# matyasosvath/hutoken

Hardware: AMD Instinct MI355X
Metric: GB/s input text encoded (GPT-2 vocab) at 1/2/4/8 GPUs; bit-exact ids (higher is better)
Workload: dtype u8

## Files before the change

hutoken_amd/_capi.py:

```python
import ctypes as C
import importlib.util
import os
import sys

from . import build as _build

OK = 0
E_FILE_NOT_FOUND, E_VALUE, E_MEMORY, E_ARG, E_DEVICE, E_UNSUPPORTED = 1, 2, 3, 4, 5, 6
E_CAPACITY, E_NUL_BYTE, E_WORD_TOO_LARGE, E_INVALID_UTF8 = 7, 8, 9, 10
DOC_OK, DOC_WORD_TOO_LARGE, DOC_INVALID_UTF8 = 0, 1, 2
DOC_ID_OUT_OF_RANGE, DOC_ID_UNDECODABLE, DOC_SPAN_MISMATCH = 3, 4, 5

_vp, _i64, _i32, _s32, _u32, _str = C.c_void_p, C.c_int64, C.c_int, C.c_int32, C.c_uint32, C.c_char_p
_pvp, _pi64, _ps32, _pf = C.POINTER(_vp), C.POINTER(_i64), C.POINTER(_s32), C.POINTER(C.c_float)
_DEV = [_vp, _vp, _vp, _i64, _i64, _vp, _i64, _vp, _vp, _vp, _vp]
_DEV_F = [_vp, _vp, _vp, _i64, _i64, _i32, _vp, _i64, _vp, _vp, _vp, _vp]
_HOST = [_vp, _vp, _vp, _i64, _vp, _i64, _vp, _vp]
_HOST_F = [_vp, _vp, _vp, _i64, _i32, _vp, _i64, _vp, _vp]
SIGNATURES = {
    "hutk_ctx_create": (_i32, [_pvp, _str, _str, _str, _i32, _i32]),
    "hutk_ctx_create_merges": (_i32, [_pvp, _str, _str, _str, _i32, _str, _i32]),
    "hutk_ctx_set_pattern": (_i32, [_vp, _str]),
    "hutk_ctx_set_pretokenizer": (_i32, [_vp, _i32, _vp, _i64]),
    "hutk_ctx_pretokenizer": (_i32, [_vp]),
    "hutk_ctx_add_device": (_i32, [_vp, _i32]),
    "hutk_ctx_device_count": (_i32, [_vp]),
    "hutk_uses_merges": (_i32, [_vp]),
    "hutk_ctx_destroy": (None, [_vp]),
    "hutk_last_error": (_str, []),
    "hutk_ids_capacity": (_i64, [_vp, _i64, _i64]),
    "hutk_encode_batch": (_i32, _HOST),
    "hutk_encode_batch_device": (_i32, _DEV),
    "hutk_encode": (_i32, [_vp, _vp, _i64, _vp, _i64, _pi64, _ps32]),
    "hutk_vocab_size": (_i64, [_vp]),
    "hutk_host_alloc": (_vp, [C.c_size_t]),
    "hutk_host_free": (None, [_vp]),
    "hutk_decode_batch": (_i32, _HOST),
    "hutk_decode_batch_device": (_i32, _DEV),
    "hutk_pair_table_entries": (_i64, [_vp]),
    "hutk_device_ordinal": (_i32, [_vp]),
    "hutk_table_stats": (_i32, [_vp, _vp]),
    "hutk_last_timing": (_i32, [_vp, _pf, _pf]),
    "hutk_set_timing": (None, [_vp, _i32]),
    "hutk_debug_pairs_second": (_i64, [_vp]),
    "hutk_debug_long_words": (_i64, [_vp]),
    "hutk_debug_profile": (_i32, [_vp, _i32]),
    "hutk_debug_profile_read": (_i32, [_vp, _i64, _vp]),
    "hutk_debug_profile_raw": (_i32, [_vp, _i64, _vp]),
    "hutk_debug_tile_bytes": (_i32, []),
    "hutk_debug_seam": (_i32, [_vp, _vp]),
    "hutk_debug_seam2_cut": (_i32, [_vp, _u32, _u32]),
    "hutk_debug_tile_kernel": (_i32, [_vp, _i64]),
    "hutk_debug_exc_counts": (_i32, [_vp, _vp]),
    "hutk_ctx_word_cache_stats": (_i32, [_vp, _vp]),
    "hutk_ctx_word_cache_clear": (_i32, [_vp]),
    "hutk_trainer_create": (_i32, [_pvp, _i32]),
    "hutk_trainer_add": (_i32, [_vp, _vp, _vp, _i64]),
    "hutk_trainer_run": (_i32, [_vp, _s32, _vp, _vp, _ps32]),
    "hutk_trainer_stats": (_i32, [_vp, _vp]),
    "hutk_trainer_destroy": (None, [_vp]),
    "hutk_trainer_debug_counters": (_i32, [_vp, _vp, _i32]),
    "hutk_trainer_create_mode": (_i32, [_pvp, _i32, _i32]),
    "hutk_trainer_alphabet": (_i32, [_vp, _vp, _i64, _vp, _i64, _pi64, _pi64]),
    "hutk_collate_padded_device": (_i32, [_vp, _vp, _i64, _i64, _i64, _s32, _s32, _s32, _i32, _i32, _vp, _vp, _vp, _vp, _vp]),
    "hutk_packer_create": (_i32, [_pvp, _i64, _s32, _s32, _s32, _i32, _i32]),
    "hutk_packer_rows": (_i64, [_vp, _i64, _i64]),
    "hutk_packer_add_device": (_i32, [_vp, _vp, _vp, _i64, _i64, _vp, _vp, _vp, _i64, _pi64, _vp, _vp]),
    "hutk_packer_flush_device": (_i32, [_vp, _vp, _vp, _vp, _pi64, _vp]),
    "hutk_packer_pending": (_i64, [_vp]),
    "hutk_packer_destroy": (None, [_vp]),
    "hutk_packer_create_channels": (_i32, [_pvp, _i64, _s32, _s32, _s32, _i32, _i32, _i32, _vp, _vp, _vp]),
    "hutk_packer_channel_count": (_i32, [_vp]),
    "hutk_packer_add_channels_device": (_i32, [_vp, _vp, _vp, _i64, _i64, _vp, _vp, _vp, _vp, _vp, _i64, _pi64, _vp, _vp]),
    "hutk_packer_flush_channels_device": (_i32, [_vp, _vp, _vp, _vp, _vp, _pi64, _vp]),
    "hutk_packed_cu_seqlens_device": (_i32, [_vp, _i64, _i64, _i64, _vp, _vp, _vp, _vp]),
    "hutk_packed_labels_device": (_i32, [_vp, _i32, _vp, _i64, _i64, _i32, _i64, _vp, _vp]),
    "hutk_debug_cu_tile": (_i32, []),
    "hutk_bestfit_rows_bound": (_i64, [_i64, _i64, _i64, _i32]),
# ... 272 lines not shown
        raise_for(load().hutk_ctx_set_pattern(self._h, None if pattern is None else pattern.encode("utf-8")))

    def set_pretokenizer(self, preset, blob=None):
        if preset is None:
            raise_for(load().hutk_ctx_set_pretokenizer(self._h, -1, None, 0))
            return
        buf = (C.c_uint8 * max(len(blob), 1)).from_buffer_copy(bytes(blob) or b"\0")
        raise_for(load().hutk_ctx_set_pretokenizer(self._h, int(preset), C.cast(buf, C.c_void_p), len(blob)))

    @property
    def pretokenizer(self):
        p = load().hutk_ctx_pretokenizer(self._h)
        return None if p < 0 else p

    @property
    def uses_merges(self):
        return bool(load().hutk_uses_merges(self._h))

    @property
    def handle(self):
        return self._h

    def ids_capacity(self, n_bytes, n_docs):
        return load().hutk_ids_capacity(self._h, n_bytes, n_docs)

    def table_stats(self):
        import numpy as np
        out = np.zeros(8, dtype=np.int64)
        raise_for(load().hutk_table_stats(self._h, out.ctypes.data))
        keys = ["n_keys", "n_vocab_sym", "n_sym", "n_pairs", "pair_slots", "rank_is_sym", "ident_ids", "n_word_entries"]
        d = dict(zip(keys, out.tolist()))
        if hasattr(load(), "hutk_debug_long_words"):
            d["n_long_word_entries"] = int(load().hutk_debug_long_words(self._h))
        return d

    def seam_map(self):
        import numpy as np
        out = np.zeros(256, dtype=np.uint32)
        on = load().hutk_debug_seam(self._h, out.ctypes.data)
        return out, bool(on)

    def seam2_cut(self, a3, b3):
        return bool(load().hutk_debug_seam2_cut(self._h, int.from_bytes(a3, "little"), int.from_bytes(b3, "little")))

    def tile_kernel(self, n_bytes):
        k = load().hutk_debug_tile_kernel(self._h, int(n_bytes))
        if k < 0:
            raise_for(E_ARG)
        return k

    def exc_counts(self):
        import numpy as np
        out = np.zeros(8, dtype=np.int64)
        raise_for(load().hutk_debug_exc_counts(self._h, out.ctypes.data))
        v = out.tolist()
        return {"exc": v[0], "lists": v[1:6], "tail": v[6], "has_multi": bool(v[7])}

    def word_cache_stats(self):
        import numpy as np
        out = np.zeros(4, dtype=np.int64)
        raise_for(load().hutk_ctx_word_cache_stats(self._h, out.ctypes.data))
        v = out.tolist()
        return {"entries": v[0], "capacity": v[1], "appended": v[2], "open": bool(v[3])}

    def word_cache_clear(self):
        raise_for(load().hutk_ctx_word_cache_clear(self._h))
# ... 816 lines not shown
```

hutoken_amd/csrc/hutk_api.cpp:

```cpp
#include <hip/hip_runtime.h>

#include <regex.h>
#if defined(__linux__)
#include <sys/syscall.h>
#include <unistd.h>
#endif

#include <algorithm>
#include <atomic>
#include <cctype>
#include <chrono>
#include <cstdio>
#include <cstdlib>
#include <cstring>
#include <mutex>
#include <new>
#include <string>
#include <thread>
#include <vector>

#include "hutk_classify.h"
#include "hutk_host.h"
constexpr int PTILES_DEFAULT = 2;

// ... 275 lines not shown
    const size_t n = T.cand_sym.size();
    if (!n) return HUTK_OK;
    std::vector<int64_t> offs(n + 1), oo(n + 1);
    for (size_t i = 0; i <= n; i++) offs[i] = T.cand_off[i];
    std::vector<int32_t> ids((size_t)hutk_ids_capacity(c, (int64_t)T.cand_bytes.size(), (int64_t)n));
    const int had_prefix = c->dt.has_prefix;
    c->dt.has_prefix = 0;
    int rc = hutk_encode_batch(c, T.cand_bytes.data(), offs.data(), (int64_t)n, ids.data(), (int64_t)ids.size(),
                               oo.data(), nullptr);
    c->dt.has_prefix = had_prefix;
    if (rc) return rc;
    const int64_t key_bytes = T.sym16 ? WORD_KEY_BYTES_16 : WORD_KEY_BYTES_32;
    std::vector<size_t> keep, keep_long;
    for (size_t i = 0; i < n; i++)
        if (oo[i + 1] - oo[i] == 1 && ids[oo[i]] == T.sym_id[T.cand_sym[i]] && offs[i + 1] - offs[i] >= 2 &&
            offs[i + 1] - offs[i] <= WORDL_KEY_BYTES)
            (offs[i + 1] - offs[i] <= key_bytes ? keep : keep_long).push_back(i);
    auto key_of = [&](size_t i, uint32_t* k) {
        for (int q = 0; q < 7; q++) k[q] = 0;
        const size_t len = (size_t)(offs[i + 1] - offs[i]);
        for (size_t j = 0; j < len; j++) k[j >> 2] |= (uint32_t)T.cand_bytes[offs[i] + j] << (8 * (j & 3));
    };
    std::vector<WordSlot> slots(1, WordSlot{{0, 0, 0, 0}});
    uint32_t cap = 0;
    if (!keep.empty()) {
        std::vector<uint4> kk(keep.size());
        for (size_t q = 0; q < keep.size(); q++) {
            uint32_t k[7];
            key_of(keep[q], k);
            kk[q] = make_uint4(k[0], k[1], k[2], k[3]);
        }
        cap = 1024;
        while (cap < keep.size() * 5 / 2 + 16) cap <<= 1;
        std::vector<uint32_t> where, homeless;
        auto hash_of = [&](uint32_t j) { const uint4 k = kk[j]; return word_hash(k.x, k.y, k.z, k.w); };
        cuckoo_place(keep.size(), cap, [&](uint32_t j) { return hash_of(j) & (cap - 1); },
                     [&](uint32_t j) { return word_slot2(hash_of(j), cap - 1); }, where, &homeless);
        slots.assign(cap + 1, WordSlot{{0, 0, 0, 0}});
        for (size_t j = 0; j < keep.size(); j++) {
            if (where[j] == 0xFFFFFFFFu) continue;
            const uint4 k = kk[j];
            slots[where[j]] = T.sym16 ? WordSlot{{k.x, k.y, k.z, k.w | (T.cand_sym[keep[j]] << 16)}}
                                      : WordSlot{{k.x, k.y, k.z, T.cand_sym[keep[j]]}};
            c->n_word_entries++;
        }
    }
    uint32_t lcap = 0, loff = 0;
    if (cap && !keep_long.empty() && !getenv("HUTK_NO_LONG_WORD_TABLE")) {
        lcap = 256;
        while (lcap < keep_long.size() * 8 + 16) lcap <<= 1;
        loff = (uint32_t)slots.size();
        loff += loff & 1u;
        slots.resize((size_t)loff + 2 * (size_t)lcap, WordSlot{{0, 0, 0, 0}});
        for (size_t j = 0; j < keep_long.size(); j++) {
            uint32_t k[7];
            key_of(keep_long[j], k);
            const size_t at = (size_t)loff + 2 * (size_t)(word_hash_long(k[0], k[1], k[2], k[3], k[4], k[5], k[6]) & (lcap - 1));
            if (slots[at].k[0] | slots[at].k[1] | slots[at].k[2] | slots[at].k[3]) continue;
            slots[at] = WordSlot{{k[0], k[1], k[2], k[3]}};
            slots[at + 1] = WordSlot{{k[4], k[5], k[6], T.cand_sym[keep_long[j]]}};
            c->n_word_entries++;
            c->n_wordl_entries++;
        }
    }
    if (!cap) return HUTK_OK;
    HUTK_HIP_TRY(c->d_word_tab.reserve(slots.size()));
    HUTK_HIP_TRY(hipMemcpy(c->d_word_tab.p, slots.data(), slots.size() * sizeof(WordSlot), hipMemcpyHostToDevice));
    c->dt.word_tab = c->d_word_tab.p;
    c->dt.word_mask = cap - 1;
    c->dt.wordl_off = loff;
// ... 113 lines not shown
        return rc;
    }
    p->pattern = c->pattern;
    if (c->presplit >= 0) {
        const int prc = hutk_pretokenizer_create(&p->pretok, device, c->presplit_blob.data(), (int64_t)c->presplit_blob.size());
        if (prc) {
            std::string keep = g_err;
            destroy(p);
            g_err = keep;
            return prc;
        }
        p->presplit = c->presplit;
    }
    c->peers.push_back(p);
    c->peer_ids.emplace_back();
    return HUTK_OK;
}

int hutk_ctx_device_count(const hutk_ctx* c) { return c && !c->host_only ? 1 + (int)c->peers.size() : 0; }

void hutk_ctx_destroy(hutk_ctx* ctx) { destroy(ctx); }

int64_t hutk_ids_capacity(const hutk_ctx* ctx, int64_t n_bytes, int64_t n_docs) {
    if (!ctx) return 0;
    return n_bytes * (int64_t)ctx->tab.max_units_per_item + (int64_t)pad_per_doc(ctx) * n_docs + 1;
}

int64_t hutk_vocab_size(const hutk_ctx* ctx) { return ctx ? ctx->tab.n_keys : 0; }
int hutk_uses_merges(const hutk_ctx* ctx) { return ctx && ctx->tab.id_path ? 1 : 0; }
int64_t hutk_pair_table_entries(const hutk_ctx* ctx) { return ctx ? ctx->tab.n_pairs : 0; }
int hutk_device_ordinal(const hutk_ctx* ctx) { return ctx ? ctx->device : -1; }
int64_t hutk_debug_pairs_second(const hutk_ctx* ctx) { return ctx ? ctx->tab.n_pairs_second : 0; }
int64_t hutk_debug_long_words(const hutk_ctx* ctx) { return ctx ? ctx->n_wordl_entries : 0; }
int hutk_debug_seam(const hutk_ctx* ctx, uint32_t* out256) {
    if (!ctx || !out256) return api_set_error(HUTK_E_ARG, "bad argument");
    memcpy(out256, ctx->tab.seam_hi, sizeof ctx->tab.seam_hi);
    return seams_wanted(ctx->tab) ? 1 : 0;
}
int hutk_debug_seam2_cut(const hutk_ctx* ctx, uint32_t a3, uint32_t b3) {
    if (!ctx) return 0;
    const Tables& T = ctx->tab;
    if (!T.seam_on || !T.seam2_on || (getenv("HUTK_NO_SEAM") && atoi(getenv("HUTK_NO_SEAM"))) ||
        (getenv("HUTK_NO_SEAM2") && atoi(getenv("HUTK_NO_SEAM2"))))
        return 0;
    if (!seam2_char3(a3) || !seam2_char3(b3)) return 0;
    if ((T.seam2_part[(a3 >> 16) & 0xFFu] >> (b3 & 31u)) & 1u) return 0;
    const uint32_t kinds[5][2] = {{3, 3}, {3, 2}, {3, 1}, {1, 3}, {1, 2}};
    for (auto& kk : kinds) {
        if (!(T.seam2_cats & seam2_cat_bit(kk[0], kk[1]))) continue;
        const uint32_t a = kk[0] == 3 ? a3 : (a3 >> 16) & 0xFFu;
        const uint32_t b = kk[1] == 3 ? b3 : kk[1] == 2 ? (b3 & 0xFFFFu) : (b3 & 0xFFu);
        const uint32_t h = seam2_hash(a, b, kk[0], kk[1]) >> T.seam2_shift;
        if ((T.seam2_bits[h >> 5] >> (h & 31)) & 1u) return 0;
    }
    return 1;
}
void hutk_set_timing(hutk_ctx* ctx, int enabled) {
    if (ctx) ctx->timing = enabled != 0;
}

int hutk_table_stats(const hutk_ctx* ctx, int64_t* out8) {
    if (!ctx || !out8) return HUTK_E_ARG;
    const Tables& T = ctx->tab;
    out8[0] = T.n_keys;
    out8[1] = T.n_vocab_sym;
    out8[2] = T.n_sym;
// ... 855 lines not shown
```

hutoken_amd/csrc/hutk_host.h:

```cpp
#pragma once
#include <hip/hip_runtime.h>

#include <mutex>
#include <string>
#include <utility>
#include <vector>

#include "hutk_device.h"

#define HUTK_HIP_TRY(expr)                                                                                  \
    do {                                                                                                    \
        hipError_t e__ = (expr);                                                                            \
        if (e__ != hipSuccess)                                                                              \
            return hutk::api_set_error(HUTK_E_DEVICE, std::string("HIP error: ") + hipGetErrorString(e__) + \
                                                          " at " #expr);                                    \
    } while (0)

namespace hutk {

template <class T>
struct DevBuf {
    T* p = nullptr;
    size_t cap = 0;
    hipError_t reserve(size_t n) {
// ... 47 lines not shown
        return HUTK_OK;
    }
    DecTables tables(bool skip) const {
        DecTables t{};
        t.ent = skip ? dx_ent_skip.p : dx_ent.p;
        t.sent = !strip ? nullptr : skip ? dx_sent_skip.p : dx_sent.p;
        t.blob = dx_blob.p;
        t.n = n;
        return t;
    }
    void release() {
        dx_ent.release(); dx_sent.release(); dx_ent_skip.release(); dx_sent_skip.release(); dx_slots.release();
        dx_blob.release();
    }
};

}

using hutk::DevBuf;

struct hutk_ctx {
    hutk::Tables tab;
    int device = -1;
    bool host_only = false;
    bool timing = true;

    DevBuf<uint64_t> d_pair, d_char;
    DevBuf<int32_t> d_sym_id, d_prefix_alone;
    DevBuf<uint32_t> d_item_sym, d_prefix_syms, d_prefix_alone_syms, d_seam, d_seam2, d_item_units;
    DevBuf<uint8_t> d_item_direct, d_split_dfa;
    DevBuf<uint32_t> d_bytepair16;
    DevBuf<hutk::WordSlot> d_word_tab;
    int64_t n_word_entries = 0, n_wordl_entries = 0;
    DevBuf<uint4> d_wc_tab, d_wc_list;
    DevBuf<uint32_t> d_wc_tags, d_wc_ctl;
    uint32_t wc_list_cap = 0;
    DevBuf<uint64_t> d_bytepair32;
    DevBuf<long long> w_prof;
    bool profile = false;
    std::string pattern;
    DevBuf<uint32_t> w_wbits, w_gbits, w_fbits, w_abits;
    int presplit = -1;
    struct hutk_pretokenizer* pretok = nullptr;
    std::vector<uint8_t> presplit_blob;
    hutk::DevTables dt{};

    DevBuf<uint32_t> w_run;
    DevBuf<int32_t> w_exc_tok;
    DevBuf<uint32_t> w_exc_sym, w_exc_mrg, w_tile_u32, w_doc_pos, w_counters;
    DevBuf<int64_t> w_tile_i64;
    DevBuf<hutk::ExcRec> w_exc;
    DevBuf<uint32_t> w_exc_quad, w_exc_mid, w_exc_wave;
    int last_tail = -1;

    DevBuf<uint2> d_dec_ent, d_dec_sent;
    DevBuf<uint8_t> d_dec_blob;
    hutk::DecTables dec{};
    DevBuf<uint32_t> dw_first;
    DevBuf<unsigned long long> dw_state;
    DevBuf<int64_t> dw_tfd;
    DevBuf<int32_t> dw_ids;
    DevBuf<int32_t> ds_ids, ds_status;
    DevBuf<int64_t> ds_offs, ds_oo;
    DevBuf<uint8_t> ds_bytes;
    DevBuf<int32_t> w_err;
    DevBuf<uint64_t> sp_bits;
// ... 270 lines not shown
```

hutoken_amd/csrc/hutk_internal.h:

```cpp
#pragma once
#include "hutk_seam2.h"
#include <cstdint>
#include <string>
#include <vector>

#include "hutoken_amd.h"

#if defined(__HIPCC__)
#include <hip/hip_runtime.h>
#define HUTK_HD __host__ __device__ __forceinline__
#else
#define HUTK_HD inline
#endif

namespace hutk {

constexpr uint32_t SYM_BITS = 20;
constexpr uint32_t SYM_UNK = (1u << SYM_BITS) - 1;
constexpr uint32_t SYM_NONE = 0xFFFFFFFFu;
constexpr uint64_t SLOT_EMPTY = ~0ull;
constexpr int WORDL_KEY_BYTES = 28;

constexpr uint32_t PAIR_ABSENT = 0xFFFFFu;
static inline uint64_t pair_slot(uint32_t l, uint32_t r, uint32_t m) {
// ... 36 lines not shown
                                std::vector<uint32_t>* failed = nullptr) {
    const uint32_t NONE = 0xFFFFFFFFu;
    std::vector<uint32_t> owner(cap, NONE);
    where.assign(n, NONE);
    bool all = true;
    uint64_t rng = 0x9E3779B97F4A7C15ull;
    for (size_t i = 0; i < n; i++) {
        uint32_t cur = (uint32_t)i;
        uint32_t slot = h1(cur) & (cap - 1);
        bool placed = false;
        for (int kick = 0; kick < 2000; kick++) {
            const uint32_t a = h1(cur) & (cap - 1), b = h2(cur) & (cap - 1);
            if (owner[a] == NONE) slot = a;
            else if (owner[b] == NONE) slot = b;
            else {
                rng = rng * 6364136223846793005ull + 1442695040888963407ull;
                slot = (slot == a) ? b : (slot == b) ? a : ((rng >> 33) & 1u ? a : b);
            }
            const uint32_t prev = owner[slot];
            owner[slot] = cur;
            where[cur] = slot;
            if (prev == NONE) { placed = true; break; }
            where[prev] = NONE;
            cur = prev;
        }
        if (!placed) {
            all = false;
            if (!failed) return false;
            failed->push_back(cur);
        }
    }
    return all;
}
HUTK_HD uint32_t char_hash(uint32_t packed) {
    uint32_t h = packed * 0x9E3779B1u;
    h ^= h >> 16;
    return h * 0x85EBCA6Bu;
}
HUTK_HD uint32_t char_slot1(uint32_t h, uint32_t shift) { return h >> shift; }
HUTK_HD uint32_t char_slot2(uint32_t h, uint32_t mask) { return ((h >> 7) ^ ((h & 0x7Fu) * 0x2F1Bu) ^ 0x5A5Au) & mask; }

constexpr int64_t MAX_WORD_BYTES = 262144;

struct Tables {
    int64_t n_keys = 0;
    uint32_t n_vocab_sym = 0;
    uint32_t n_sym = 0;
    bool rank_is_sym = false;
    bool ident_ids = false;
    std::vector<int32_t> sym_id;
    int32_t byte_tok[256] = {0};

    std::vector<uint64_t> pair_slots;
    uint32_t pair_shift = 0;
    int64_t n_pairs = 0;
    int64_t n_pairs_second = 0;

    uint32_t item_sym[256];
    uint8_t item_direct[256];
    uint32_t multi_bits[8] = {0, 0, 0, 0, 0, 0, 0, 0};
    uint32_t item_units_off[257] = {0};
    std::vector<uint32_t> item_units;
    uint32_t max_units_per_item = 1;
    bool has_multi = false;
    std::vector<uint64_t> char_slots;
    uint32_t char_mask = 0;
// ... 59 lines not shown
```

hutoken_amd/csrc/hutk_kernels.hip:

```cpp
#include <hip/hip_runtime.h>

#include <type_traits>

#include "hutk_kdev.h"
#include "hutk_lab.h"

namespace hutk {

__device__ __noinline__ void cut_note_cold(uint32_t* noreal_bits, uint32_t* counters, uint32_t tile, unsigned long long mine,
                                                  uint32_t last16, uint32_t* cutpos) {
    if ((threadIdx.x & 63) != 0) return;
    if (mine == 0) {
        atomicOr(&noreal_bits[tile >> 5], 1u << (tile & 31));
        atomicAdd(&counters[CTR_NOREAL_TILES], 1u);
    } else {
        *cutpos = 1u + (uint32_t)(16 * (63 - __builtin_clzll(mine)) + 31 - __builtin_clz(last16 & 0xFFFFu));
    }
}

struct Win8 { uint32_t d[8]; };
__device__ __noinline__ uint32_t classify16_exact_cold(Win8 w, uint32_t dbits, uint32_t* tmp) {
#pragma unroll
    for (int i = 0; i < 8; i++) tmp[i] = w.d[i];
    return classify16_exact(*reinterpret_cast<const uint32_t(*)[8]>(tmp), dbits);
// ... 46 lines not shown
template <typename SymT, bool BYTE_MODE>
struct TileLds {
    static constexpr int ARENA_WORDS = 4, ARENA_W = LANE_MAX_UNITS + 4;
    __attribute__((aligned(16))) uint8_t sb[WINDOW];
    uint32_t docm[WINDOW / 32 + 3];
    __attribute__((aligned(8))) uint16_t wmask16[64 + 8];
    __attribute__((aligned(8))) uint32_t mergem[NPOS / 32 + 2];
    __attribute__((aligned(8))) uint32_t excm[NPOS / 32 + 2];
    __attribute__((aligned(8))) uint32_t livem[NPOS / 32 + 2];
    uint16_t stage[64];
    __attribute__((aligned(16))) SymT S[NPOS];
    SymT arenaS[BYTE_MODE ? 1 : ARENA_WORDS * ARENA_W];
    SymT arenaM[BYTE_MODE ? 1 : ARENA_WORDS * ARENA_W];
    uint32_t arena_live[ARENA_WORDS];
    uint16_t arena_ws[ARENA_WORDS], arena_n[ARENA_WORDS];
    uint32_t arena_used, extra;
    uint32_t cutpos;
};

template <typename RunT>
__device__ __forceinline__ void d_gather(const DevTables& T, const BatchArgs& A, const Workspace& W, int64_t vwave);
__device__ __forceinline__ void d_doc_off(const BatchArgs& A, const Workspace& W, int64_t vblock);

template <typename SymT, bool BYTE_MODE, bool RANK_IS_SYM, int WAVES, bool MULTI = false, bool ONE = false>
__global__ __launch_bounds__(64 * WAVES) __attribute__((amdgpu_waves_per_eu(sizeof(SymT) == 2 ? (BYTE_MODE ? (RANK_IS_SYM ? TILE_WAVES_EU : 7) : TILE_CHAR_EU) : 3))) void k_tiles(DevTables T, BatchArgs A_in, Workspace W) {
    BatchArgs A = A_in;
    typedef TileLds<SymT, BYTE_MODE> Tile;
    constexpr int ARENA_WORDS = Tile::ARENA_WORDS, ARENA_W = Tile::ARENA_W;
    constexpr int POOL_CAP = 64 * WAVES;
    constexpr int POOL_LONG_CAP = POOL_CAP * 3 / 8, POOL_LONG = 8;
    static_assert(WAVES <= 32, "pool entries keep the tile-in-workgroup index in 6 bits");
    constexpr bool FAST_TRIPS = RANK_IS_SYM && sizeof(SymT) == 2;
    constexpr bool WCACHE = BYTE_MODE && FAST_TRIPS && !MULTI;
    __shared__ Tile L[WAVES];
    __shared__ uint32_t pool_cnt[3];
    __shared__ uint32_t s_exc_cnt;
    __shared__ unsigned long long s_exc_base;
    __shared__ SymT s_item_sym[BYTE_MODE ? 2 : 256];
    __shared__ uint32_t s_item_direct[BYTE_MODE ? 1 : 8];
    constexpr int M_ARENA = 352 * WAVES + 192;
    struct MergeLds {
        __attribute__((aligned(16))) SymT m[M_ARENA];
        uint32_t pool[POOL_CAP];
    };
    struct SplitLds {
        uint8_t dfa[dfa::TABLE_BYTES];
        uint8_t lut[256];
    };
    __shared__ __attribute__((aligned(16))) union {
        MergeLds g;
        SplitLds c;
    } s_m;
    static_assert(M_ARENA >= 2 * LANE_MAX_UNITS, "arena size");
    uint32_t* const pool = s_m.g.pool;
#if HUTK_LAB_LDS_PAD
    __shared__ uint32_t s_lab_pad[HUTK_LAB_LDS_PAD / 4];
    if (A.n_docs < 0) s_lab_pad[threadIdx.x] = 1;
#endif

    if (select_skips(W, A.n_tiles)) return;
    if constexpr (ONE) {
        const size_t off_bytes = (((size_t)A.n_docs + 1) * 8 + 15) & ~(size_t)15;
        const size_t n16 = (off_bytes + (size_t)A.n_bytes + 15) / 16;
        const uint4* src = reinterpret_cast<const uint4*>(A.offsets);
        uint4* dst = reinterpret_cast<uint4*>(W.one_in);
        for (size_t i = threadIdx.x; i < n16; i += 64 * WAVES) dst[i] = src[i];
// ... 302 lines not shown
                        __builtin_memcpy(&key, sb + LOOKBACK + ws, 16);
                        const uint32_t isym = T.item_sym[key.x & 0xFFu];
                        const uint64_t mlo = nb >= 8 ? ~0ull : ((1ull << (8 * nb)) - 1ull);
                        const uint64_t mhi = nb <= 8 ? 0ull : ((1ull << (8 * (nb - 8))) - 1ull);
                        const uint32_t k0 = key.x & (uint32_t)mlo, k1 = key.y & (uint32_t)(mlo >> 32);
                        const uint32_t k2 = key.z & (uint32_t)mhi, k3 = key.w & (uint32_t)(mhi >> 32);
                        bool done = nb == 1;
                        uint32_t sym = isym;
                        if (T.word_mask) {
                            const uint32_t wh = word_hash(k0, k1, k2, k3);
                            uint4 s1 = reinterpret_cast<const uint4*>(T.word_tab)[wh & T.word_mask];
                            uint4 s2 = reinterpret_cast<const uint4*>(T.word_tab)[word_slot2(wh, T.word_mask)];
                            asm volatile("" : "+v"(s1.x), "+v"(s2.x));
                            const uint32_t d1 = KSH == 32 ? 0u : (s1.w ^ k3) << (KSH & 31);
                            const uint32_t d2 = KSH == 32 ? 0u : (s2.w ^ k3) << (KSH & 31);
                            const bool hit1 = ((s1.x ^ k0) | (s1.y ^ k1) | (s1.z ^ k2) | d1) == 0;
                            const bool hit2 = ((s2.x ^ k0) | (s2.y ^ k1) | (s2.z ^ k2) | d2) == 0;
                            if (nb != 1 && (hit1 || hit2)) {
                                const uint32_t swd = hit1 ? s1.w : s2.w;
                                sym = KSH == 32 ? swd : swd >> (KSH & 31);
                                done = true;
                            }
                        }
                        if (done) {
                            S[ws] = Sym<SymT>::narrow(sym);
                        } else {
                            atomicOr(&mergem[ws >> 5], 1u << (ws & 31));
                        }
                    }
                    wave_sync();
                }
            }
        }
        uint32_t nW;
        const uint32_t wbase = wave_excl_scan(__popc(rest), lane, &nW);
        uint32_t widx = wbase;
        for (uint32_t r0 = 0; r0 < nW; r0 += 64) {
            while (rest && widx - r0 < 64u) {
                stage[widx - r0] = (uint16_t)(16 * lane + __builtin_ctz(rest));
                rest &= rest - 1;
                widx++;
            }
            wave_sync();
            if (r0 + lane < nW) {
                const int ws = stage[lane];
                const uint64_t nxt = bits64(wmask32, ws + 1) & 0x7FFFFFFFFFFFFFFFull;
                const int nb = nxt ? 1 + __builtin_ctzll(nxt) : 64;
                const bool known_end = nxt != 0 && (ws + nb < NPOS || t0 + ws + nb >= A.n_bytes);
                const bool docfirst = bit_at(docm, ws + LOOKBACK);
                const uint32_t b0 = sb[ws + LOOKBACK];
                const bool gap = A.gap_bits && ((A.gap_bits[(t0 + ws) >> 5] >> ((t0 + ws) & 31)) & 1u);
                const bool sp0 = A.alone_bits ? gbit(A.alone_bits, t0 + ws) : b0 == ' ';
                const bool pfx = !gap && T.has_prefix && docfirst && !sp0;
                bool exc = !gap && (!known_end || nb > LANE_MAX_BYTES || (BYTE_MODE && T.has_prefix && docfirst));
                if (MULTI && !gap && !exc) {
                    bool m = false;
                    for (int i = 0; i < nb; i++) {
                        const uint32_t b = sb[ws + LOOKBACK + i];
                        if (BYTE_MODE || !is_cont(b)) m = m || ((T.multi_bits[b >> 5] >> (b & 31u)) & 1u);
                    }
                    exc = m;
                }
                if (!BYTE_MODE && !exc && T.has_prefix && docfirst && !pfx)
                    exc = atomicAdd(&s_extra, (uint32_t)T.n_prefix_alone) + T.n_prefix_alone > (uint32_t)RUN_EXTRA;
                constexpr int WORD_KEY = sizeof(SymT) == 2 ? WORD_KEY_BYTES_16 : WORD_KEY_BYTES_32;
                const bool probe = !gap && !exc && !pfx && T.word_mask && nb >= 2 && nb <= WORD_KEY;
                uint32_t k0, k1, k2, k3;
                {
                    const int a = (ws + LOOKBACK) & ~3, o8 = 8 * ((ws + LOOKBACK) & 3);
                    const uint32_t* sw = reinterpret_cast<const uint32_t*>(sb + a);
                    const uint32_t q0 = sw[0], q1 = sw[1], q2 = sw[2], q3 = sw[3], q4 = sw[4];
                    k0 = funnel_r(q1, q0, o8);
                    k1 = funnel_r(q2, q1, o8);
                    k2 = funnel_r(q3, q2, o8);
                    k3 = funnel_r(q4, q3, o8);
                    const uint64_t mlo = nb >= 8 ? ~0ull : ((1ull << (8 * nb)) - 1ull);
                    const uint64_t mhi = nb <= 8 ? 0ull : nb >= 16 ? ~0ull : ((1ull << (8 * (nb - 8))) - 1ull);
                    k0 &= (uint32_t)mlo;
                    k1 &= (uint32_t)(mlo >> 32);
                    k2 &= (uint32_t)mhi;
                    k3 &= (uint32_t)(mhi >> 32);
                }
                const bool probe_long = !gap && !exc && !pfx && T.wordl_mask && nb > WORD_KEY && nb <= WORDL_KEY_BYTES;
                uint32_t k4 = 0, k5 = 0, k6 = 0;
                const uint32_t wh = word_hash(k0, k1, k2, k3);
                uint32_t o1 = probe ? wh & T.word_mask : 0u;
                uint32_t o2 = probe ? word_slot2(wh, T.word_mask) : 0u;
                if (__any(probe_long)) {
                    if (probe_long) {
                        const int a = (ws + LOOKBACK) & ~3, o8 = 8 * ((ws + LOOKBACK) & 3);
                        const uint32_t* sw = reinterpret_cast<const uint32_t*>(sb + a);
                        const uint32_t q4 = sw[4], q5 = sw[5], q6 = sw[6], q7 = sw[7];
                        const int nb2 = nb - 16;
                        const uint64_t mlo = nb2 >= 8 ? ~0ull : nb2 <= 0 ? 0ull : ((1ull << (8 * nb2)) - 1ull);
                        const uint32_t mhi = nb2 <= 8 ? 0u : nb2 >= 12 ? ~0u : ((1u << (8 * (nb2 - 8))) - 1u);
                        k4 = funnel_r(q5, q4, o8) & (uint32_t)mlo;
                        k5 = funnel_r(q6, q5, o8) & (uint32_t)(mlo >> 32);
                        k6 = funnel_r(q7, q6, o8) & mhi;
                        o1 = T.wordl_off + 2u * (word_hash_long(k0, k1, k2, k3, k4, k5, k6) & T.wordl_mask);
                        o2 = o1 + 1u;
                    }
                }
                uint4 s1 = make_uint4(0, 0, 0, 0), s2 = s1;
                uint32_t isym = 0;
                if (T.word_mask) {
                    s1 = reinterpret_cast<const uint4*>(T.word_tab)[o1];
                    s2 = reinterpret_cast<const uint4*>(T.word_tab)[o2];
                }
                if (BYTE_MODE) isym = T.item_sym[b0];
#if HUTK_PERTURB_MEM
                {
                    uint32_t acc = 0;
#pragma unroll
                    for (int j = 0; j < HUTK_PERTURB_MEM; j++) {
                        const uint4 v = T.pair_buckets[(wh * (2u * j + 3u) * 0x9E3779B1u) >> T.pair_shift];
                        acc ^= v.x ^ v.w;
                    }
                    if (acc == 0x12345678u && wh == 0x9E3779B9u) raise(A.err, HUTK_E_MEMORY);
                }
#endif
                bool done = false;
                if (probe) {
                    constexpr int KSH = sizeof(SymT) == 2 ? 16 : 32;
                    const uint32_t d1 = KSH == 32 ? 0u : (s1.w ^ k3) << (KSH & 31);
                    const uint32_t d2 = KSH == 32 ? 0u : (s2.w ^ k3) << (KSH & 31);
                    const bool hit1 = ((s1.x ^ k0) | (s1.y ^ k1) | (s1.z ^ k2) | d1) == 0;
                    const bool hit2 = ((s2.x ^ k0) | (s2.y ^ k1) | (s2.z ^ k2) | d2) == 0;
                    done = hit1 || hit2;
                    const uint32_t sw = hit1 ? s1.w : s2.w;
                    if (done) S[ws] = Sym<SymT>::narrow(KSH == 32 ? sw : sw >> (KSH & 31));
                }
                if (probe_long) {
                    done = ((s1.x ^ k0) | (s1.y ^ k1) | (s1.z ^ k2) | (s1.w ^ k3) | (s2.x ^ k4) | (s2.y ^ k5) | (s2.z ^ k6)) == 0;
                    if (done) S[ws] = Sym<SymT>::narrow(s2.w);
                }
                int n = 0;
                SymT* Sdst = S + ws;
                int slot = -1;
                if (!BYTE_MODE && !exc && pfx) {
                    slot = (int)atomicAdd(&s_arena_used, 1u);
                    if (slot >= ARENA_WORDS ||
                        atomicAdd(&s_extra, (uint32_t)T.n_prefix) + T.n_prefix > (uint32_t)RUN_EXTRA) exc = true;
                    else {
                        Sdst = arenaS + slot * ARENA_W;
                        for (int i = 0; i < T.n_prefix && i < ARENA_W; i++) Sdst[i] = Sym<SymT>::narrow(T.prefix_syms[i]);
                        n = T.n_prefix;
                    }
                }
                const int n_cap = pfx ? ARENA_W : LANE_MAX_UNITS;
                if (!gap && !exc && !done) {
                    if (BYTE_MODE) {
                        n = nb;
                    } else {
                        const int lw = ws + LOOKBACK;
                        int i = 0;
                        while (i < nb) {
                            const uint32_t b = sb[lw + i];
                            int L = 1;
                            if (b >= 0x80u) {
                                L = (b >= 0xF0u) ? 4 : (b >= 0xE0u) ? 3 : (b >= 0xC0u) ? 2 : 1;
// ... 17 lines not shown
                }
                if (gap) {
                    atomicAnd(&livem[ws >> 5], ~(1u << (ws & 31)));
                    done = true;
                } else if (done) {
                } else if (!BYTE_MODE && !exc && pfx) {
                    arena_ws[slot] = (uint16_t)ws;
                    arena_n[slot] = (uint16_t)n;
                    atomicAnd(&livem[ws >> 5], ~(1u << (ws & 31)));
                } else if (exc) {
                    atomicOr(&excm[ws >> 5], 1u << (ws & 31));
                    atomicAnd(&livem[ws >> 5], ~(1u << (ws & 31)));
                    done = true;
                } else if (n == 1) {
                    if (BYTE_MODE) S[ws] = Sym<SymT>::narrow(isym);
                    done = true;
                }
                if (!done) atomicOr(&mergem[ws >> 5], 1u << (ws & 31));
            }
            wave_sync();
        }
        HUTK_STAMP(4);
        {
            const uint32_t e16 = reinterpret_cast<const uint16_t*>(excm)[lane];
            if (__any(e16 != 0)) {
                uint32_t tot;
                (void)wave_excl_scan((uint32_t)__popc(e16), lane, &tot);
                uint32_t off = 0;
                if (lane == 0) off = atomicAdd(&s_exc_cnt, tot | (1u << 16));
                my_exc_off = (uint32_t)__builtin_amdgcn_readfirstlane((int)off);
            }
        }

        if constexpr (WCACHE) {
            if (T.wc_on) {
                uint32_t pend = reinterpret_cast<const uint16_t*>(mergem)[lane];
                uint32_t nP;
                uint32_t pidx = wave_excl_scan((uint32_t)__popc(pend), lane, &nP);
                for (uint32_t r0 = 0; r0 < nP; r0 += 64) {
                    while (pend && pidx - r0 < 64u) {
                        stage[pidx - r0] = (uint16_t)(16 * lane + __builtin_ctz(pend));
                        pend &= pend - 1;
                        pidx++;
                    }
                    wave_sync();
                    if (r0 + lane < nP) {
                        const int ws = stage[lane];
                        const int nb = word_units(me, ws);
                        if (nb >= wc::MIN_BYTES && nb <= wc::KEY_BYTES) {
                            uint32_t k[wc::KEY_DWORDS];
                            wc_key(me, ws, nb, k);
                            const uint4* line = T.wc_tab + (size_t)wc::bucket_of(wc::hash(k), T.wc_log2) * 8u;
                            uint4 a0 = line[0], a1 = line[1], b0 = line[4], b1 = line[5];
                            asm volatile("" : "+v"(a0.x), "+v"(a1.x), "+v"(b0.x), "+v"(b1.x));
                            const uint32_t s1[wc::KEY_DWORDS] = {a0.x, a0.y, a0.z, a0.w, a1.x, a1.y, a1.z, a1.w};
                            const uint32_t s2[wc::KEY_DWORDS] = {b0.x, b0.y, b0.z, b0.w, b1.x, b1.y, b1.z, b1.w};
                            const bool hit1 = wc::key_hit(s1, k), hit2 = wc::key_hit(s2, k);
                            if (hit1 || hit2) {
                                const uint4* sy = line + (hit1 ? 2 : 6);
                                const uint4 y0 = sy[0], y1 = sy[1];
                                const int n = wc::slot_n(hit1 ? a1.w : b1.w);
                                const uint32_t y[8] = {y0.x, y0.y, y0.z, y0.w, y1.x, y1.y, y1.z, y1.w};
#pragma unroll
                                for (int i = 0; i < wc::MAX_IDS; i++)
                                    if (i < n) S[ws + i] = (SymT)(y[i >> 1] >> (16 * (i & 1)));
                                const uint64_t lm = (uint64_t)(((1u << n) - 1u) & ~1u) << (ws & 31);
                                if ((uint32_t)lm) atomicOr(&livem[ws >> 5], (uint32_t)lm);
                                if ((uint32_t)(lm >> 32)) atomicOr(&livem[(ws >> 5) + 1], (uint32_t)(lm >> 32));
                                atomicAnd(&mergem[ws >> 5], ~(1u << (ws & 31)));
                            }
                        }
                    }
                    wave_sync();
                }
            }
        }
    }

#if HUTK_ABLATE_MERGE
    if (tile_ok) reinterpret_cast<uint16_t*>(mergem)[lane] = 0;
#endif
#if HUTK_PERTURB_SLEEP
    for (int i = 0; i < HUTK_PERTURB_SLEEP; i++) __builtin_amdgcn_s_sleep(127);
#endif
    [[maybe_unused]] bool first_epoch = true;
    for (;;) {
#if HUTK_MERGE_STAMPS
        if (first_epoch && tile_ok && W.prof && lane == 0)
            W.prof[tile * N_PHASE + 0] = (clock64() & ~3ll) | (long long)__builtin_amdgcn_s_getreg((1 << 11) | (4 << 6) | 4);
#endif
        if (threadIdx.x == 0) { pool_cnt[0] = 0; pool_cnt[1] = 0; pool_cnt[2] = FAST_TRIPS ? 2u : 0u; }
// ... 1108 lines not shown
```

include/hutoken_amd.h:

```cpp
#ifndef HUTOKEN_AMD_H
#define HUTOKEN_AMD_H

#include <stddef.h>
#include <stdint.h>

#ifdef __cplusplus
extern "C" {
#endif

typedef struct hutk_ctx hutk_ctx;

enum {
    HUTK_OK = 0,
    HUTK_E_FILE_NOT_FOUND = 1,
    HUTK_E_VALUE = 2,
    HUTK_E_MEMORY = 3,
    HUTK_E_ARG = 4,
    HUTK_E_DEVICE = 5,
    HUTK_E_UNSUPPORTED = 6,
    HUTK_E_CAPACITY = 7,
    HUTK_E_NUL_BYTE = 8,
    HUTK_E_WORD_TOO_LARGE = 9,
    HUTK_E_INVALID_UTF8 = 10
};
// ... 31 lines not shown


int hutk_encode_batch_device(hutk_ctx* ctx, const uint8_t* d_bytes, const int64_t* d_offsets,
                             int64_t n_docs, int64_t n_bytes, int32_t* d_ids_out,
                             int64_t ids_cap, int64_t* d_out_offsets, int32_t* d_status,
                             int32_t* d_err, void* hip_stream);

void* hutk_host_alloc(size_t n_bytes);
void hutk_host_free(void* p);

int hutk_encode(hutk_ctx* ctx, const uint8_t* text, int64_t len, int32_t* ids_out,
                int64_t ids_cap, int64_t* n_ids, int32_t* status);

int hutk_decode_batch(hutk_ctx* ctx, const int32_t* ids, const int64_t* id_offsets, int64_t n_docs,
                      uint8_t* bytes_out, int64_t bytes_cap, int64_t* out_offsets, int32_t* status);
int hutk_decode_batch_device(hutk_ctx* ctx, const int32_t* d_ids, const int64_t* d_id_offsets,
                             int64_t n_docs, int64_t n_ids, uint8_t* d_bytes_out, int64_t bytes_cap,
                             int64_t* d_out_offsets, int32_t* d_status, int32_t* d_err, void* hip_stream);

int64_t hutk_vocab_size(const hutk_ctx* ctx);
int64_t hutk_pair_table_entries(const hutk_ctx* ctx);
int hutk_uses_merges(const hutk_ctx* ctx);
int hutk_device_ordinal(const hutk_ctx* ctx);
int hutk_table_stats(const hutk_ctx* ctx, int64_t* out8);

int hutk_ctx_word_cache_stats(hutk_ctx* ctx, int64_t* out4);
int hutk_ctx_word_cache_clear(hutk_ctx* ctx);

int hutk_last_timing(hutk_ctx* ctx, float* ms_tile_kernel, float* ms_total);

int64_t hutk_debug_pairs_second(const hutk_ctx* ctx);

int64_t hutk_debug_long_words(const hutk_ctx* ctx);

int hutk_debug_seam(const hutk_ctx* ctx, uint32_t* out256);
int hutk_debug_seam2_cut(const hutk_ctx* ctx, uint32_t a3, uint32_t b3);
int hutk_debug_tile_kernel(const hutk_ctx* ctx, int64_t n_bytes);
int hutk_debug_exc_counts(const hutk_ctx* ctx, int64_t* out8);

int hutk_debug_profile(hutk_ctx* ctx, int enable);
int hutk_debug_tile_bytes(void);
int hutk_debug_profile_read(hutk_ctx* ctx, int64_t n_tiles, double* out10);
int hutk_debug_profile_raw(hutk_ctx* ctx, int64_t n_tiles, long long* out);

void hutk_set_timing(hutk_ctx* ctx, int enabled);

#define HUTK_TRAIN_BYTES 0
#define HUTK_TRAIN_CHARS 1
typedef struct hutk_trainer hutk_trainer;
int hutk_trainer_create(hutk_trainer** out, int device);
int hutk_trainer_create_mode(hutk_trainer** out, int device, int mode);
int hutk_trainer_alphabet(hutk_trainer* t, uint8_t* bytes_out, int64_t bytes_cap, int64_t* offsets_out,
                          int64_t offsets_cap, int64_t* n_symbols, int64_t* n_bytes);
int hutk_trainer_add(hutk_trainer* t, const uint8_t* bytes, const int64_t* offsets, int64_t n_docs);
int hutk_trainer_run(hutk_trainer* t, int32_t n_merges, int32_t* pairs_out, int64_t* counts_out, int32_t* n_done);
int hutk_trainer_stats(const hutk_trainer* t, int64_t* out8);
int hutk_trainer_debug_counters(const hutk_trainer* t, int64_t* out, int n);
void hutk_trainer_destroy(hutk_trainer* t);

#define HUTK_COLLATE_TRUNC_LEFT 1
#define HUTK_COLLATE_PAD_LEFT 2
#define HUTK_NO_TOKEN INT32_MIN
int hutk_collate_padded_device(const int32_t* d_ids, const int64_t* d_offsets, int64_t n_docs, int64_t n_ids,
                               int64_t max_len, int32_t bos_id, int32_t eos_id, int32_t pad_id, int flags,
                               int out_width, void* d_input_ids, uint8_t* d_mask, int32_t* d_lengths, int32_t* d_err,
                               void* hip_stream);
// ... 276 lines not shown
```

Before: 284.5.

## Probe word table first slot only, defer second-slot probe to pending pass

On the host, the word hash table is built with a cuckoo placement that prefers first-choice slots. On the device, a new batched path probes only the first slot for short words, with three rounds of loads in flight, and marks misses as pending. The second-slot probe is moved into the later pending pass alongside the word cache. The aim is to cut global memory traffic per word, since most words should resolve in their first slot. The cost is added kernel complexity and extra work for words that land in their second slot.

Result: no change. 286.9 (median of 6 runs) (+0.9%).

```diff
diff --git a/hutoken_amd/_capi.py b/hutoken_amd/_capi.py
--- a/hutoken_amd/_capi.py
+++ b/hutoken_amd/_capi.py
@@ -44,6 +44,7 @@
     "hutk_set_timing": (None, [_vp, _i32]),
     "hutk_debug_pairs_second": (_i64, [_vp]),
     "hutk_debug_long_words": (_i64, [_vp]),
+    "hutk_debug_words_second": (_i64, [_vp]),
     "hutk_debug_profile": (_i32, [_vp, _i32]),
     "hutk_debug_profile_read": (_i32, [_vp, _i64, _vp]),
     "hutk_debug_profile_raw": (_i32, [_vp, _i64, _vp]),
@@ -382,6 +383,8 @@
         d = dict(zip(keys, out.tolist()))
         if hasattr(load(), "hutk_debug_long_words"):
             d["n_long_word_entries"] = int(load().hutk_debug_long_words(self._h))
+        if hasattr(load(), "hutk_debug_words_second"):
+            d["n_word_second"] = int(load().hutk_debug_words_second(self._h))
         return d
 
     def seam_map(self):
diff --git a/hutoken_amd/csrc/hutk_api.cpp b/hutoken_amd/csrc/hutk_api.cpp
--- a/hutoken_amd/csrc/hutk_api.cpp
+++ b/hutoken_amd/csrc/hutk_api.cpp
@@ -331,10 +331,13 @@
         }
         cap = 1024;
         while (cap < keep.size() * 5 / 2 + 16) cap <<= 1;
-        std::vector<uint32_t> where, homeless;
-        auto hash_of = [&](uint32_t j) { const uint4 k = kk[j]; return word_hash(k.x, k.y, k.z, k.w); };
-        cuckoo_place(keep.size(), cap, [&](uint32_t j) { return hash_of(j) & (cap - 1); },
-                     [&](uint32_t j) { return word_slot2(hash_of(j), cap - 1); }, where, &homeless);
+        std::vector<uint32_t> where, homeless, s1(keep.size()), s2(keep.size());
+        for (size_t j = 0; j < keep.size(); j++) {
+            const uint32_t h = word_hash(kk[j].x, kk[j].y, kk[j].z, kk[j].w);
+            s1[j] = h & (cap - 1);
+            s2[j] = word_slot2(h, cap - 1);
+        }
+        c->n_word_second = (int64_t)word_table_place(s1, s2, cap, where, &homeless);
         slots.assign(cap + 1, WordSlot{{0, 0, 0, 0}});
         for (size_t j = 0; j < keep.size(); j++) {
             if (where[j] == 0xFFFFFFFFu) continue;
@@ -514,6 +517,7 @@
 int hutk_device_ordinal(const hutk_ctx* ctx) { return ctx ? ctx->device : -1; }
 int64_t hutk_debug_pairs_second(const hutk_ctx* ctx) { return ctx ? ctx->tab.n_pairs_second : 0; }
 int64_t hutk_debug_long_words(const hutk_ctx* ctx) { return ctx ? ctx->n_wordl_entries : 0; }
+int64_t hutk_debug_words_second(const hutk_ctx* ctx) { return ctx ? ctx->n_word_second : 0; }
 int hutk_debug_seam(const hutk_ctx* ctx, uint32_t* out256) {
     if (!ctx || !out256) return api_set_error(HUTK_E_ARG, "bad argument");
     memcpy(out256, ctx->tab.seam_hi, sizeof ctx->tab.seam_hi);
diff --git a/hutoken_amd/csrc/hutk_host.h b/hutoken_amd/csrc/hutk_host.h
--- a/hutoken_amd/csrc/hutk_host.h
+++ b/hutoken_amd/csrc/hutk_host.h
@@ -103,6 +103,7 @@
     DevBuf<uint32_t> d_bytepair16;
     DevBuf<hutk::WordSlot> d_word_tab;
     int64_t n_word_entries = 0, n_wordl_entries = 0;
+    int64_t n_word_second = 0;
     DevBuf<uint4> d_wc_tab, d_wc_list;
     DevBuf<uint32_t> d_wc_tags, d_wc_ctl;
     uint32_t wc_list_cap = 0;
diff --git a/hutoken_amd/csrc/hutk_internal.h b/hutoken_amd/csrc/hutk_internal.h
--- a/hutoken_amd/csrc/hutk_internal.h
+++ b/hutoken_amd/csrc/hutk_internal.h
@@ -92,6 +92,69 @@
     }
     return all;
 }
+static inline size_t word_table_place(const std::vector<uint32_t>& s1, const std::vector<uint32_t>& s2, uint32_t cap,
+                                      std::vector<uint32_t>& where, std::vector<uint32_t>* failed = nullptr,
+                                      std::vector<uint8_t>* why = nullptr) {
+    const uint32_t NONE = 0xFFFFFFFFu;
+    const size_t n = s1.size();
+    std::vector<uint32_t> where0, failed0;
+    cuckoo_place(n, cap, [&](uint32_t j) { return s1[j]; }, [&](uint32_t j) { return s2[j]; }, where0, &failed0);
+    std::vector<uint8_t> later(n, 0);
+    for (uint32_t j : failed0) later[j] = 1;
+    std::vector<uint32_t> owner(cap, NONE);
+    std::vector<uint32_t> homeless;
+    where.assign(n, NONE);
+    if (why) why->assign(n, 0);
+    uint64_t rng = 0x9E3779B97F4A7C15ull;
+    bool lost = false;
+    for (size_t i = 0; i < n && !lost; i++) {
+        if (later[i]) continue;
+        uint32_t cur = (uint32_t)i;
+        uint32_t from = NONE;
+        bool placed = false;
+        for (int kick = 0; kick < 2000; kick++) {
+            const uint32_t a = s1[cur], b = s2[cur];
+            uint32_t slot;
+            if (owner[a] == NONE) slot = a;
+            else if (owner[b] == NONE) slot = b;
+            else if (from == a) slot = b;
+            else if (from == b) slot = a;
+            else {
+                const bool a2 = s2[owner[a]] == a, b2 = s2[owner[b]] == b;
+                rng = rng * 6364136223846793005ull + 1442695040888963407ull;
+                slot = a2 != b2 ? (a2 ? a : b) : ((rng >> 33) & 1u ? a : b);
+            }
+            if (why && from == NONE && owner[a] != NONE) (*why)[cur] |= 1u;
+            const uint32_t prev = owner[slot];
+            owner[slot] = cur;
+            where[cur] = slot;
+            if (prev == NONE) { placed = true; break; }
+            where[prev] = NONE;
+            if (why) (*why)[prev] |= 2u;
+            cur = prev;
+            from = slot;
+        }
+        lost = !placed;
+    }
+    if (lost) {
+        where = where0;
+        homeless = failed0;
+        if (why)
+            for (size_t j = 0; j < n; j++) (*why)[j] = where[j] != NONE && where[j] == s2[j] ? 2u : 0u;
+    } else {
+        for (uint32_t j : failed0) {
+            const uint32_t slot = owner[s1[j]] == NONE ? s1[j] : owner[s2[j]] == NONE ? s2[j] : NONE;
+            if (slot == NONE) { homeless.push_back(j); continue; }
+            owner[slot] = j;
+            where[j] = slot;
+            if (why && slot == s2[j]) (*why)[j] |= 1u;
+        }
+    }
+    if (failed) *failed = homeless;
+    size_t second = 0;
+    for (size_t j = 0; j < n; j++) second += where[j] != NONE && where[j] == s2[j];
+    return second;
+}
 HUTK_HD uint32_t char_hash(uint32_t packed) {
     uint32_t h = packed * 0x9E3779B1u;
     h ^= h >> 16;
diff --git a/hutoken_amd/csrc/hutk_kernels.hip b/hutoken_amd/csrc/hutk_kernels.hip
--- a/hutoken_amd/csrc/hutk_kernels.hip
+++ b/hutoken_amd/csrc/hutk_kernels.hip
@@ -102,6 +102,7 @@
     static_assert(WAVES <= 32, "pool entries keep the tile-in-workgroup index in 6 bits");
     constexpr bool FAST_TRIPS = RANK_IS_SYM && sizeof(SymT) == 2;
     constexpr bool WCACHE = BYTE_MODE && FAST_TRIPS && !MULTI;
+    constexpr bool PROBE1 = BYTE_MODE && !MULTI && !ONE && sizeof(SymT) == 2;
     __shared__ Tile L[WAVES];
     __shared__ uint32_t pool_cnt[3];
     __shared__ uint32_t s_exc_cnt;
@@ -470,6 +471,79 @@
                 }
             }
         }
+        if constexpr (PROBE1) {
+            if (!A.word_bits && T.word_mask) {
+                constexpr int PK = 3;
+                const uint32_t f32 = flags | ((uint32_t)wmask16[lane + 1] << 16);
+                uint32_t x = f32 >> 1;
+                x |= x >> 1;
+                x |= x >> 2;
+                x |= x >> 4;
+                x |= x >> (WORD_KEY_BYTES_16 - 8);
+                uint32_t shorts = own & x;
+                if (T.has_prefix) shorts &= ~(uint32_t)bits64(docm, 16 * lane + LOOKBACK);
+                rest = own & ~shorts;
+                uint32_t nS;
+                uint32_t sidx = wave_excl_scan(__popc(shorts), lane, &nS);
+                for (uint32_t r0 = 0; r0 < nS; r0 += 64u * PK) {
+                    uint32_t wsn[PK];
+                    uint32_t kk[PK][4];
+                    uint4 sv[PK];
+                    uint32_t iv[PK];
+#pragma unroll
+                    for (int j = 0; j < PK; j++) {
+                        wsn[j] = 0xFFFFFFFFu;
+                        sv[j] = make_uint4(0, 0, 0, 0);
+                        iv[j] = 0;
+                        kk[j][0] = kk[j][1] = kk[j][2] = kk[j][3] = 0;
+                        const uint32_t base = r0 + 64u * (uint32_t)j;
+                        if (base < nS) {
+                            while (shorts && sidx - base < 64u) {
+                                stage[sidx - base] = (uint16_t)(16 * lane + __builtin_ctz(shorts));
+                                shorts &= shorts - 1;
+                                sidx++;
+                            }
+                            wave_sync();
+                            const bool mine = base + lane < nS;
+                            uint32_t nb = 0, b0 = 0;
+                            if (mine) {
+                                const uint32_t ws = stage[lane];
+                                nb = 1u + (uint32_t)__builtin_ctzll(bits64(wmask32, ws + 1));
+                                const int a = (ws + LOOKBACK) & ~3, o8 = 8 * ((ws + LOOKBACK) & 3);
+                                const uint32_t* sw = reinterpret_cast<const uint32_t*>(sb + a);
+                                const uint32_t q0 = sw[0], q1 = sw[1], q2 = sw[2], q3 = sw[3], q4 = sw[4];
+                                const uint64_t mlo = nb >= 8 ? ~0ull : ((1ull << (8 * nb)) - 1ull);
+                                const uint64_t mhi = nb <= 8 ? 0ull : ((1ull << (8 * (nb - 8))) - 1ull);
+                                kk[j][0] = funnel_r(q1, q0, o8) & (uint32_t)mlo;
+                                kk[j][1] = funnel_r(q2, q1, o8) & (uint32_t)(mlo >> 32);
+                                kk[j][2] = funnel_r(q3, q2, o8) & (uint32_t)mhi;
+                                kk[j][3] = funnel_r(q4, q3, o8) & (uint32_t)(mhi >> 32);
+                                b0 = kk[j][0] & 0xFFu;
+                                wsn[j] = ws | (nb << 16);
+                                if (nb >= 2)
+                                    sv[j] = reinterpret_cast<const uint4*>(T.word_tab)[word_hash(kk[j][0], kk[j][1], kk[j][2], kk[j][3]) & T.word_mask];
+                            }
+                            if (__any(nb == 1)) {
+                                if (nb == 1) iv[j] = T.item_sym[b0];
+                            }
+                            wave_sync();
+                        }
+                    }
+                    asm volatile("" : "+v"(sv[0].x), "+v"(sv[1].x), "+v"(sv[2].x));
+                    static_assert(PK == 3, "the line above names every sub-round's load");
+#pragma unroll
+                    for (int j = 0; j < PK; j++) {
+                        if (wsn[j] != 0xFFFFFFFFu) {
+                            const uint32_t ws = wsn[j] & 0xFFFFu, nb = wsn[j] >> 16;
+                            const bool hit = ((sv[j].x ^ kk[j][0]) | (sv[j].y ^ kk[j][1]) | (sv[j].z ^ kk[j][2]) | ((sv[j].w ^ kk[j][3]) << 16)) == 0;
+                            if (nb == 1) S[ws] = Sym<SymT>::narrow(iv[j]);
+                            else if (hit) S[ws] = (SymT)(sv[j].w >> 16);
+                            else atomicOr(&mergem[ws >> 5], 1u << (ws & 31));
+                        }
+                    }
+                }
+            }
+        }
         uint32_t nW;
         const uint32_t wbase = wave_excl_scan(__popc(rest), lane, &nW);
         uint32_t widx = wbase;
@@ -523,8 +597,9 @@
                 uint32_t k4 = 0, k5 = 0, k6 = 0;
                 const uint32_t wh = word_hash(k0, k1, k2, k3);
                 uint32_t o1 = probe ? wh & T.word_mask : 0u;
-                uint32_t o2 = probe ? word_slot2(wh, T.word_mask) : 0u;
-                if (__any(probe_long)) {
+                uint32_t o2 = probe && !PROBE1 ? word_slot2(wh, T.word_mask) : 0u;
+                const bool any_long = __any(probe_long);
+                if (any_long) {
                     if (probe_long) {
                         const int a = (ws + LOOKBACK) & ~3, o8 = 8 * ((ws + LOOKBACK) & 3);
                         const uint32_t* sw = reinterpret_cast<const uint32_t*>(sb + a);
@@ -543,9 +618,19 @@
                 uint32_t isym = 0;
                 if (T.word_mask) {
                     s1 = reinterpret_cast<const uint4*>(T.word_tab)[o1];
-                    s2 = reinterpret_cast<const uint4*>(T.word_tab)[o2];
-                }
-                if (BYTE_MODE) isym = T.item_sym[b0];
+                    if constexpr (PROBE1) {
+                        if (any_long) {
+                            if (probe_long) s2 = reinterpret_cast<const uint4*>(T.word_tab)[o2];
+                        }
+                    } else {
+                        s2 = reinterpret_cast<const uint4*>(T.word_tab)[o2];
+                    }
+                }
+                if constexpr (PROBE1) {
+                    if (__any(nb == 1)) {
+                        if (nb == 1) isym = T.item_sym[b0];
+                    }
+                } else if (BYTE_MODE) isym = T.item_sym[b0];
 #if HUTK_PERTURB_MEM
                 {
                     uint32_t acc = 0;
@@ -563,7 +648,7 @@
                     const uint32_t d1 = KSH == 32 ? 0u : (s1.w ^ k3) << (KSH & 31);
                     const uint32_t d2 = KSH == 32 ? 0u : (s2.w ^ k3) << (KSH & 31);
                     const bool hit1 = ((s1.x ^ k0) | (s1.y ^ k1) | (s1.z ^ k2) | d1) == 0;
-                    const bool hit2 = ((s2.x ^ k0) | (s2.y ^ k1) | (s2.z ^ k2) | d2) == 0;
+                    const bool hit2 = !PROBE1 && ((s2.x ^ k0) | (s2.y ^ k1) | (s2.z ^ k2) | d2) == 0;
                     done = hit1 || hit2;
                     const uint32_t sw = hit1 ? s1.w : s2.w;
                     if (done) S[ws] = Sym<SymT>::narrow(KSH == 32 ? sw : sw >> (KSH & 31));
@@ -647,8 +732,11 @@
             }
         }
 
-        if constexpr (WCACHE) {
-            if (T.wc_on) {
+        if constexpr (WCACHE || PROBE1) {
+            bool wc_on = false;
+            if constexpr (WCACHE) wc_on = T.wc_on != 0;
+            const bool tab_on = PROBE1 && T.word_mask != 0;
+            if (wc_on || tab_on) {
                 uint32_t pend = reinterpret_cast<const uint16_t*>(mergem)[lane];
                 uint32_t nP;
                 uint32_t pidx = wave_excl_scan((uint32_t)__popc(pend), lane, &nP);
@@ -662,16 +750,30 @@
                     if (r0 + lane < nP) {
                         const int ws = stage[lane];
                         const int nb = word_units(me, ws);
-                        if (nb >= wc::MIN_BYTES && nb <= wc::KEY_BYTES) {
+                        const bool cached = wc_on && nb >= wc::MIN_BYTES && nb <= wc::KEY_BYTES;
+                        const bool probe2 = tab_on && nb <= WORD_KEY_BYTES_16;
+                        if (cached || probe2) {
                             uint32_t k[wc::KEY_DWORDS];
                             wc_key(me, ws, nb, k);
-                            const uint4* line = T.wc_tab + (size_t)wc::bucket_of(wc::hash(k), T.wc_log2) * 8u;
-                            uint4 a0 = line[0], a1 = line[1], b0 = line[4], b1 = line[5];
-                            asm volatile("" : "+v"(a0.x), "+v"(a1.x), "+v"(b0.x), "+v"(b1.x));
+                            const uint4 z4 = make_uint4(0, 0, 0, 0);
+                            const uint4* line = nullptr;
+                            uint4 a0 = z4, a1 = z4, b0 = z4, b1 = z4, t2 = z4;
+                            if constexpr (WCACHE) {
+                                if (cached) {
+                                    line = T.wc_tab + (size_t)wc::bucket_of(wc::hash(k), T.wc_log2) * 8u;
+                                    a0 = line[0]; a1 = line[1]; b0 = line[4]; b1 = line[5];
+                                }
+                            }
+                            if (probe2) t2 = reinterpret_cast<const uint4*>(T.word_tab)[word_slot2(word_hash(k[0], k[1], k[2], k[3]), T.word_mask)];
+                            asm volatile("" : "+v"(a0.x), "+v"(a1.x), "+v"(b0.x), "+v"(b1.x), "+v"(t2.x));
+                            const bool hit_tab = probe2 && ((t2.x ^ k[0]) | (t2.y ^ k[1]) | (t2.z ^ k[2]) | ((t2.w ^ k[3]) << 16)) == 0;
                             const uint32_t s1[wc::KEY_DWORDS] = {a0.x, a0.y, a0.z, a0.w, a1.x, a1.y, a1.z, a1.w};
                             const uint32_t s2[wc::KEY_DWORDS] = {b0.x, b0.y, b0.z, b0.w, b1.x, b1.y, b1.z, b1.w};
-                            const bool hit1 = wc::key_hit(s1, k), hit2 = wc::key_hit(s2, k);
-                            if (hit1 || hit2) {
+                            const bool hit1 = cached && !hit_tab && wc::key_hit(s1, k), hit2 = cached && !hit_tab && wc::key_hit(s2, k);
+                            if (hit_tab) {
+                                S[ws] = (SymT)(t2.w >> 16);
+                                atomicAnd(&mergem[ws >> 5], ~(1u << (ws & 31)));
+                            } else if (hit1 || hit2) {
                                 const uint4* sy = line + (hit1 ? 2 : 6);
                                 const uint4 y0 = sy[0], y1 = sy[1];
                                 const int n = wc::slot_n(hit1 ? a1.w : b1.w);
diff --git a/include/hutoken_amd.h b/include/hutoken_amd.h
--- a/include/hutoken_amd.h
+++ b/include/hutoken_amd.h
@@ -87,6 +87,8 @@
 int64_t hutk_debug_pairs_second(const hutk_ctx* ctx);
 
 int64_t hutk_debug_long_words(const hutk_ctx* ctx);
+
+int64_t hutk_debug_words_second(const hutk_ctx* ctx);
 
 int hutk_debug_seam(const hutk_ctx* ctx, uint32_t* out256);
 int hutk_debug_seam2_cut(const hutk_ctx* ctx, uint32_t a3, uint32_t b3);
```
